# RenYurui/Global-Flow-Local-Attention

Measured on AMD Instinct MI355X. Metric: images/sec (fwd+bwd) PoseGenerator 256x176 attn_layer=2,3 -- feature-warping hot path, higher is better.
Workload: dtype f32 (FC products: 2-term f16 splits exact to 2^-24 on f16 MFMA, f32 accumulate)

## Files before the change

### global_flow_local_attention_amd/_lib.py

```python
import ctypes
import os
import subprocess

import torch

_PKG = os.path.dirname(os.path.abspath(__file__))
LIB_PATH = os.environ.get("GFLA_HIP_LIBRARY") or os.path.join(_PKG, "libgfla_hip.so")
_lib = None

_i64, _int, _ptr = ctypes.c_int64, ctypes.c_int, ctypes.c_void_p

_SIGNATURES = {
    "gfla_block_extractor_fwd": [_ptr] * 3 + [_i64] * 6 + [_int, _ptr],
    "gfla_block_extractor_bwd": [_ptr] * 5 + [_i64] * 6 + [_int, _ptr],
    "gfla_block_extractor_unfold_fwd": [_ptr] * 3 + [_i64] * 6 + [_int, _int, _ptr],
    "gfla_block_extractor_unfold_bwd": [_ptr] * 5 + [_i64] * 6 + [_int, _int, _ptr],
    "gfla_local_attn_reshape_fwd": [_ptr] * 2 + [_i64] * 3 + [_int, _ptr],
    "gfla_local_attn_reshape_bwd": [_ptr] * 2 + [_i64] * 3 + [_int, _ptr],
    "gfla_resample2d_fwd": [_ptr] * 3 + [_i64] * 6 + [_int, _int, _ptr],
    "gfla_resample2d_bwd": [_ptr] * 5 + [_i64] * 6 + [_int, _int, _int, _ptr],
    "gfla_local_attn_aggregate_fwd": [_ptr] * 5 + [_i64] * 6 + [_int, _int, _ptr],
    "gfla_local_attn_aggregate_bwd": [_ptr] * 7 + [_i64] * 6 + [_int, _int, _ptr],
    "gfla_local_attn_source_bwd": [_ptr] * 7 + [_i64] * 6 + [_int, _int, _ptr],
}
_SINGLE = {
    "gfla_max_cosine_fwd_f32": [_ptr] * 5 + [_i64] * 4 + [ctypes.c_double, _ptr],
    "gfla_max_cosine_fwd_f16": [_ptr] * 5 + [_i64] * 4 + [ctypes.c_double, _ptr],
    "gfla_max_cosine_fwd_bf16": [_ptr] * 5 + [_i64] * 4 + [ctypes.c_double, _ptr],
    "gfla_max_cosine_workspace_bytes": [_i64] * 3,
    "gfla_fc_tail_fwd_f32": [_ptr, _i64, _i64] + [_ptr] * 5 + [_i64] * 3 + [_int, ctypes.c_double, _ptr],
    "gfla_fc_tail_fwd_f64": [_ptr, _i64, _i64] + [_ptr] * 5 + [_i64] * 3 + [_int, ctypes.c_double, _ptr],
    "gfla_fc_tail_bwd_f32": [_ptr, _i64, _i64] + [_ptr] * 8 + [_i64] * 3 + [_int, ctypes.c_double, _ptr],
    "gfla_fc_tail_bwd_f64": [_ptr, _i64, _i64] + [_ptr] * 8 + [_i64] * 3 + [_int, ctypes.c_double, _ptr],
    "gfla_replicate_pad_bwd_f32": [_ptr] * 2 + [_i64] * 3 + [_int] * 4 + [_ptr],
    "gfla_replicate_pad_bwd_f64": [_ptr] * 2 + [_i64] * 3 + [_int] * 4 + [_ptr],
    "gfla_correctness_map_fwd_f32": [_ptr] * 5 + [_i64] * 3 + [ctypes.c_double] * 2 + [_ptr],
    "gfla_correctness_map_bwd_f32": [_ptr] * 9 + [_i64] * 3 + [ctypes.c_double] * 2 + [_ptr],
    "gfla_correctness_map_fwd_f16": [_ptr] * 5 + [_i64] * 3 + [ctypes.c_double] * 2 + [_ptr],
    "gfla_correctness_map_bwd_f16": [_ptr] * 9 + [_i64] * 3 + [ctypes.c_double] * 2 + [_ptr],
    "gfla_correctness_map_fwd_bf16": [_ptr] * 5 + [_i64] * 3 + [ctypes.c_double] * 2 + [_ptr],
    "gfla_correctness_map_bwd_bf16": [_ptr] * 9 + [_i64] * 3 + [ctypes.c_double] * 2 + [_ptr],
    "gfla_fc_supported": [_i64] * 3 + [_int, _int],
    "gfla_fc_workspace_bytes": [_i64] * 4 + [_int] * 3,
    "gfla_fc_forward_f32": [_ptr] * 9 + [_i64] * 4 + [_int, ctypes.c_double, _int, _ptr],
    "gfla_fc_backward_f32": [_ptr] * 12 + [_i64] * 4 + [_int, ctypes.c_double, _int, _int, _ptr],
    "gfla_fc_geometry": [_i64, _i64, _int, _int, _ptr],
    "gfla_fc_conv_fwd_f32": [_ptr, _ptr, _int, _ptr, _ptr] + [_i64] * 4 + [_int, _int, _ptr],
    "gfla_fc_conv_bwd_f32": [_ptr, _int, _ptr, _ptr, _ptr, _ptr] + [_i64] * 4 + [_int, _int, _ptr],
    "gfla_fc_tr_probe": [_ptr, _int, _ptr, _ptr, _ptr],
    "gfla_fc_wino_debug_buffer": [_ptr],
    "gfla_fc_kernel_f32": [_int, _ptr, _ptr] + [_i64] * 4 + [_int, _int, _ptr],
    "gfla_scatter_workspace_bytes": [_i64] * 3 + [_int],
    "gfla_aggregate_fwd_workspace_bytes": [_i64] * 3 + [_int],
    "gfla_aggregate_fwd_geometry": [_i64] * 6 + [_int, _ptr],
    "gfla_aggregate_bwd_supported": [_i64, _i64, _int],
    "gfla_big_plane_geometry": [_int] + [_i64] * 6 + [_int, _int, _ptr],
    "gfla_xcd_swizzle": [_i64, _i64],
    "gfla_local_attn_aggregate_fwd_ws_f32": [_ptr] * 6 + [_i64] * 6 + [_int, _int, _ptr],
    "gfla_local_attn_aggregate_fwd_ws_bf16": [_ptr] * 6 + [_i64] * 6 + [_int, _int, _ptr],
    "gfla_local_attn_aggregate_fwd_ws_f16": [_ptr] * 6 + [_i64] * 6 + [_int, _int, _ptr],
    "gfla_local_attn_aggregate_bwd_ws_f32": [_ptr] * 8 + [_i64] * 6 + [_int, _int, _ptr],
    "gfla_resample2d_bwd_ws_f32": [_ptr] * 6 + [_i64] * 6 + [_int, _int, _int, _ptr],
    "gfla_convert_multi": [_ptr, _ptr, _i64] * 4 + [_int, _ptr],
    "gfla_mask_blend_fwd_f32": [_ptr] * 6 + [_i64] * 3 + [_ptr],
    "gfla_mask_blend_fwd_bf16": [_ptr] * 6 + [_i64] * 3 + [_ptr],
    "gfla_mask_blend_bwd_f32": [_ptr] * 11 + [_i64] * 3 + [_ptr],
    "gfla_mask_blend_bwd_bf16": [_ptr] * 11 + [_i64] * 3 + [_ptr],
    "gfla_mask_blend_fwd_f16": [_ptr] * 6 + [_i64] * 3 + [_ptr],
    "gfla_mask_blend_bwd_f16": [_ptr] * 11 + [_i64] * 3 + [_ptr],
    "gfla_fc_forward_f16": [_ptr] * 9 + [_i64] * 4 + [_int, ctypes.c_double, _ptr],
    "gfla_gemm_f64_workspace_bytes": [_i64] * 3 + [_int],
    "gfla_gemm_f64": [_ptr] * 6 + [_i64] * 3 + [_int, _int, _ptr, _ptr],
    "gfla_affine_reg_workspace_bytes": [_i64] * 3 + [_int],
    "gfla_affine_reg_fwd_f32": [_ptr] * 3 + [_i64] * 3 + [_int, _ptr],
    "gfla_affine_reg_fwd_f64": [_ptr] * 3 + [_i64] * 3 + [_int, _ptr],
    "gfla_affine_reg_fwd_f16": [_ptr] * 3 + [_i64] * 3 + [_int, _ptr],
    "gfla_affine_reg_fwd_bf16": [_ptr] * 3 + [_i64] * 3 + [_int, _ptr],
    "gfla_affine_reg_bwd_f32": [_ptr] * 4 + [_i64] * 3 + [_int, _ptr],
    "gfla_affine_reg_bwd_f64": [_ptr] * 4 + [_i64] * 3 + [_int, _ptr],
    "gfla_affine_reg_bwd_f16": [_ptr] * 4 + [_i64] * 3 + [_int, _ptr],
    "gfla_affine_reg_bwd_bf16": [_ptr] * 4 + [_i64] * 3 + [_int, _ptr],
}
# ... 162 lines not shown
```

### global_flow_local_attention_amd/csrc/fc_block.hip

```cpp
#include "fc_gemm.h"

namespace gfla {

static int64_t align256(int64_t v) { return (v + 255) & ~(int64_t)255; }

enum { kAmaxSrc = 0, kAmaxTgt = 1, kAmaxW = 2, kAmaxZs = 3, kAmaxZt = 4, kAmaxSlots = 8 };

enum FcConv {
  kConvDirect,
  kConvDirect16,
  kConvWino32,
  kConvWino16,
};
enum FcWgrad {
  kWgradDirect32,
  kWgradDirect16,
  kWgradWino32,
  kWgradWino16,
};
static bool fc_wgrad_wino(FcWgrad w) { return w == kWgradWino32 || w == kWgradWino16; }

struct FcPlan {
  int split;
  bool scaled;
  FcConv fwd, dgrad;
  bool pack_wf, pack_wd;
  int pack_split;
  bool pack_uf, pack_ud;
  bool dgrads_together;
  FcWgrad wgrad;
  FcWgrad wgrad_both;
  bool wgrads_together;
  bool wgrad_x32;
// ... 527 lines not shown
  const bool unpack = L.plan.wgrad == kWgradDirect16;
  if (grad_w0 && !unpack &&
      hipMemsetAsync(grad_w0, 0, (size_t)kFcHidden * 2 * C * k * k * 4, stream) != hipSuccess)
    return GFLA_ERR_LAUNCH;
  GFLA_TRY(fc_half_backward(L, is_source != 0, ws, sc, grad_x, grad_w0, B, C, H, W, k, FcHalfCall(), stream));
  if (grad_w0 && unpack) GFLA_TRY(fc_unpack_wgrad_both(L, ws, sc, grad_w0, C, k, stream));
  return GFLA_OK;
}

int gfla_fc_kernel_f32(int which, void *workspace, void *scratch, int64_t B, int64_t C_, int64_t H_, int64_t W_,
                       int kernel_size, int mode, gfla_stream_t stream_) {
  if (!workspace || !scratch) return GFLA_ERR_NULL_POINTER;
  if (which < 0 || which > 8 || (which > 5 && !fc_is_wino(mode))) return GFLA_ERR_BAD_SHAPE;
  const int C = (int)C_, H = (int)H_, W = (int)W_, k = kernel_size;
  GFLA_TRY(fc_args_ok(B, C, H, W, k, mode));
  if (B == 0) return GFLA_OK;
  hipStream_t stream = static_cast<hipStream_t>(stream_);
  const FcLayout L = fc_layout(B, C, H, W, k, mode);
  unsigned char *ws = static_cast<unsigned char *>(workspace), *sc = static_cast<unsigned char *>(scratch);
  const bool src = which == 6 || which == 7 || (which & 1) == 0, tgt = which > 5 || (which & 1) == 1;
  float *gs = reinterpret_cast<float *>(ws + L.gs), *gt = reinterpret_cast<float *>(ws + L.gt);
  switch (which) {
    case 0: case 1: case 6: return fc_fwd_convs(L, ws, src ? gs : nullptr, tgt ? gt : nullptr, B, k, stream);
    case 2: case 3: case 7: return fc_dgrad_convs(L, ws, sc, src, tgt, B, C, k, stream);
    case 4: case 5: return fc_wgrad_half(L, src, ws, sc, B, k, stream);
    default: return fc_wgrad_wino(L.plan.wgrad_both) ? fc_wgrad_both(L, ws, sc, B, k, stream) : GFLA_ERR_UNSUPPORTED;
  }
}

int gfla_fc_tr_probe(const int16_t *image, int n_halves, const int32_t *offsets, int16_t *out, gfla_stream_t stream) {
  if (!image || !offsets || !out) return GFLA_ERR_NULL_POINTER;
  return fc_tr_probe(image, n_halves, offsets, out, static_cast<hipStream_t>(stream));
}
}
```

### global_flow_local_attention_amd/csrc/fc_wino.hip

```cpp
#include "fc_wino_shared.h"

namespace gfla {



template <int KS>
__global__ __launch_bounds__(256) void fc_wino_pack_w_kernel(const float *__restrict__ w0, WnPackJobs jobs, int C) {
  const WnPackJob jb = jobs.j[blockIdx.y];
  const int nch = (jb.n_in + kFcChunk - 1) / kFcChunk, ntn = (jb.n_out + kWnN - 1) / kWnN;
  const int64_t idx = (int64_t)blockIdx.x * 256 + threadIdx.x;
  if (!jb.U || idx >= (int64_t)ntn * kWnN * nch * kFcChunk) return;
  const int co = (int)(idx % (ntn * kWnN)), ci = (int)(idx / (ntn * kWnN));
  float w[KS][KS];
#pragma unroll
  for (int i = 0; i < KS; ++i)
#pragma unroll
    for (int j = 0; j < KS; ++j) {
      float v = 0.f;
      if (ci < jb.n_in && co < jb.n_out) {
        v = jb.dgrad ? w0[(((int64_t)ci * 2 * C + jb.c_off + co) * KS + (KS - 1 - i)) * KS + (KS - 1 - j)]
                     : w0[(((int64_t)co * 2 * C + jb.c_off + ci) * KS + i) * KS + j];
      }
      w[i][j] = v;
    }
// ... 450 lines not shown
#pragma unroll
  for (int a6 = 0; a6 < 6; ++a6) {
    if constexpr (M == 2) {
      const float a = t[a6][0], b = t[a6][1];
      zh[a6 * 6 + 0] = a, zh[a6 * 6 + 1] = a + b, zh[a6 * 6 + 2] = a - b, zh[a6 * 6 + 3] = a + 2.f * b;
      zh[a6 * 6 + 4] = a - 0.5f * b, zh[a6 * 6 + 5] = b;
    } else {
      const float a = t[a6][0], b = t[a6][1], c = t[a6][2], d = t[a6][3];
      zh[a6 * 6 + 0] = a;
      zh[a6 * 6 + 1] = a + b + c + d;
      zh[a6 * 6 + 2] = a - b + c - d;
      zh[a6 * 6 + 3] = a + 2.f * b + 4.f * c + 8.f * d;
      zh[a6 * 6 + 4] = a - 0.5f * b + 0.25f * c - 0.125f * d;
      zh[a6 * 6 + 5] = d;
    }
  }
}

struct WwUnit {
  int64_t b;
  int ty, tx0, ntx;
  int nt;
};

struct WwKArgs {
  PackedDesc X;
  const float *Z;
  float *part;
  int64_t z_bs, z_lead, total_units, SX;
  int Wp, Wo, nsplit;
  WwGeo geo;
};
template <int KS, int DBG = 0, bool MR = false>
__global__ __launch_bounds__(kWnThreads, 2) void fc_wino_wgrad_kernel(WwKArgs a0, WwKArgs a1, int nsplit0, int cpad,
                                                                     int raw_stride) {
  const bool second = (int)blockIdx.y >= nsplit0;
#define GFLA_PICK(f) (second ? a1.f : a0.f)
  PackedDesc X;
  X.base = GFLA_PICK(X.base), X.split_stride = 0, X.batch_stride = GFLA_PICK(X.batch_stride);
  X.chunk_stride = GFLA_PICK(X.chunk_stride), X.pix_stride = GFLA_PICK(X.pix_stride);
  const float *__restrict__ Z = GFLA_PICK(Z);
  float *__restrict__ part = GFLA_PICK(part);
  const int64_t z_bs = GFLA_PICK(z_bs), z_lead = GFLA_PICK(z_lead), total_units = GFLA_PICK(total_units), SX = GFLA_PICK(SX);
  const int Wp = GFLA_PICK(Wp), Wo = GFLA_PICK(Wo), nsplit = GFLA_PICK(nsplit);
  WwGeo geo;
  geo.TH = GFLA_PICK(geo.TH), geo.TW = GFLA_PICK(geo.TW), geo.nseg = GFLA_PICK(geo.nseg);
  geo.R = GFLA_PICK(geo.R), geo.ups = GFLA_PICK(geo.ups);
#undef GFLA_PICK
  constexpr int M = Ww<KS>::M, SEG = Ww<KS>::SEG, L = Ww<KS>::L, PITCH = kWwPitch;
  const int RAW = MR ? raw_stride : Ww<KS>::RAW;
  constexpr int PF1 = (6 * L * 4 + kWnThreads - 1) / kWnThreads;
  constexpr int PF = MR ? (PF1 > Ww<KS>::PFM ? PF1 : Ww<KS>::PFM) : PF1;
  extern __shared__ __attribute__((aligned(16))) unsigned char gfla_smem[];
  float *vbuf = reinterpret_cast<float *>(gfla_smem);
  unsigned char *raw = gfla_smem + 2 * kWwVFloats * 4;
  const int t = threadIdx.x, lane = t & 63, wave = t >> 6, xh = wave >> 2;
  const int cc = blockIdx.x, sp = (int)blockIdx.y - (second ? nsplit0 : 0);
  const int64_t u0 = total_units * sp / nsplit, u1 = total_units * (sp + 1) / nsplit;
  const int per_sample = geo.ups;
  const int Lr = (MR && geo.R > 1) ? M * geo.TW + 6 - M : L;
  const int raw_rows = (MR && geo.R > 1) ? M * geo.R + 6 - M : 6;
  const int npieces = raw_rows * Lr * 4;
  const unsigned inv_ntx = (65536u + (unsigned)geo.TW - 1u) / (unsigned)geo.TW;

  f32x4v acc[kWnXi];
#pragma unroll
  for (int q = 0; q < kWnXi; ++q) acc[q] = f32x4v{0.f, 0.f, 0.f, 0.f};

  auto unit_of = [&](int64_t u) {
    WwUnit un;
    un.b = u / per_sample;
    const int r = (int)(u - un.b * per_sample);
    if (MR && geo.R > 1) {
      un.ty = r * geo.R;
      un.tx0 = 0;
      un.ntx = geo.TW;
      un.nt = geo.TW * min(geo.R, geo.TH - un.ty);
    } else {
      un.ty = r / geo.nseg;
      un.tx0 = (r - un.ty * geo.nseg) * SEG;
      un.ntx = min(SEG, geo.TW - un.tx0);
      un.nt = un.ntx;
    }
    return un;
  };
  auto tile_rc = [&](int t_, int &tr, int &tcol) {
    if (MR && geo.R > 1) {
      tr = (int)(((unsigned)t_ * inv_ntx) >> 16);
      tcol = t_ - tr * geo.TW;
    } else {
// ... 220 lines not shown
constexpr int kWw16Pitch = 80;
constexpr int kWn16HeadZ = 4;
constexpr int kWw16VBytes = kWnXi * 4 * 16 * 16;

__device__ __forceinline__ void wn16_split_halves(float v, _Float16 &h, _Float16 &l) {
  asm("" : "+v"(v));
  h = (_Float16)v;
  float rem;
  asm("v_fma_mix_f32 %0, %1, 1.0, -%2 op_sel_hi:[0,0,1]" : "=v"(rem) : "v"(v), "v"(h));
  l = (_Float16)rem;
}
__device__ __forceinline__ void wn16_split_pair(float v0, float v1, uint32_t &hi, uint32_t &lo) { fc_split_pair(v0, v1, hi, lo); }
template <int A6>
__device__ __forceinline__ float ww_lift2(float a, float b) {
  if constexpr (A6 == 0) return a;
  else if constexpr (A6 == 1) return a + b;
  else if constexpr (A6 == 2) return a - b;
  else if constexpr (A6 == 3) return fmaf(2.f, b, a);
  else if constexpr (A6 == 4) return fmaf(-0.5f, b, a);
  else return b;
}

template <int A6>
__device__ __forceinline__ f32x2v ww_lift2v(f32x2v a, f32x2v b) {
  if constexpr (A6 == 0) return a;
  else if constexpr (A6 == 1) return a + b;
  else if constexpr (A6 == 2) return a - b;
  else if constexpr (A6 == 3) return __builtin_elementwise_fma(f32x2v{2.f, 2.f}, b, a);
  else if constexpr (A6 == 4) return __builtin_elementwise_fma(f32x2v{-0.5f, -0.5f}, b, a);
  else return b;
}

template <bool MR, int DBG = 0>
__global__ __launch_bounds__(kWnThreads, 2) void fc_wino16_wgrad_kernel(WwKArgs a0, WwKArgs a1, int nsplit0, int cpad,
                                                                       int raw_stride, const uint32_t *__restrict__ amax_x0,
                                                                       const uint32_t *__restrict__ amax_x1,
                                                                       const uint32_t *__restrict__ amax_z0,
                                                                       const uint32_t *__restrict__ amax_z1) {
  constexpr int KS = 5;
  const bool second = (int)blockIdx.y >= nsplit0;
#define GFLA_PICK(f) (second ? a1.f : a0.f)
  PackedDesc X;
  X.base = GFLA_PICK(X.base), X.split_stride = 0, X.batch_stride = GFLA_PICK(X.batch_stride);
  X.chunk_stride = GFLA_PICK(X.chunk_stride), X.pix_stride = GFLA_PICK(X.pix_stride);
  const float *__restrict__ Z = GFLA_PICK(Z);
  float *__restrict__ part = GFLA_PICK(part);
  const int64_t z_bs = GFLA_PICK(z_bs), z_lead = GFLA_PICK(z_lead), total_units = GFLA_PICK(total_units), SX = GFLA_PICK(SX);
  const int Wp = GFLA_PICK(Wp), nsplit = GFLA_PICK(nsplit);
  WwGeo geo;
  geo.TH = GFLA_PICK(geo.TH), geo.TW = GFLA_PICK(geo.TW), geo.nseg = GFLA_PICK(geo.nseg);
  geo.R = GFLA_PICK(geo.R), geo.ups = GFLA_PICK(geo.ups);
#undef GFLA_PICK
  const int ex = wn16_scale_exp(second ? *amax_x1 : *amax_x0, kWn16HeadX), ez = wn16_scale_exp(second ? *amax_z1 : *amax_z0, kWn16HeadZ);
  const float sx = wn16_pow2(ex), sz = wn16_pow2(ez), inv_x = wn16_pow2(254 - ex), inv_z = wn16_pow2(254 - ez);
  constexpr int M = 2, SEG = Ww<KS>::SEG, L = Ww<KS>::L, PITCH = kWw16Pitch;
  constexpr int RAW1 = (6 * L * PITCH + 15) & ~15;
  const int RAW = MR ? raw_stride : RAW1;
  constexpr int PF1 = (6 * L * 4 + kWnThreads - 1) / kWnThreads;
  constexpr int PF = MR ? (PF1 > Ww<KS>::PFM ? PF1 : Ww<KS>::PFM) : PF1;
  extern __shared__ __attribute__((aligned(16))) unsigned char gfla_smem[];
  unsigned char *vbuf = gfla_smem;
  unsigned char *raw = gfla_smem + 2 * kWw16VBytes;
  const int t = threadIdx.x, lane = t & 63, wave = t >> 6, xh = wave >> 2;
  const int cc = blockIdx.x, sp = (int)blockIdx.y - (second ? nsplit0 : 0);
  const int64_t u0 = total_units * sp / nsplit, u1 = total_units * (sp + 1) / nsplit;
  const int per_sample = geo.ups;
  const int Lr = (MR && geo.R > 1) ? M * geo.TW + 6 - M : L;
  const int raw_rows = (MR && geo.R > 1) ? M * geo.R + 6 - M : 6;
  const int npieces = raw_rows * Lr * 4;
  const unsigned inv_ntx = (65536u + (unsigned)geo.TW - 1u) / (unsigned)geo.TW;

  f32x4v acc[kWnXi];
#pragma unroll
  for (int q = 0; q < kWnXi; ++q) acc[q] = f32x4v{0.f, 0.f, 0.f, 0.f};

  auto unit_of = [&](int64_t u) {
    WwUnit un;
    un.b = u / per_sample;
    const int r = (int)(u - un.b * per_sample);
    if (MR && geo.R > 1) {
      un.ty = r * geo.R;
      un.tx0 = 0;
      un.ntx = geo.TW;
      un.nt = geo.TW * min(geo.R, geo.TH - un.ty);
    } else {
      un.ty = r / geo.nseg;
      un.tx0 = (r - un.ty * geo.nseg) * SEG;
      un.ntx = min(SEG, geo.TW - un.tx0);
      un.nt = un.ntx;
    }
    return un;
  };
  auto tile_rc = [&](int t_, int &tr, int &tcol) {
    if (MR && geo.R > 1) {
      tr = (int)(((unsigned)t_ * inv_ntx) >> 16);
      tcol = t_ - tr * geo.TW;
    } else {
// ... 257 lines not shown
  g.ups = g.R > 1 ? (g.TH + g.R - 1) / g.R : g.TH * g.nseg;
  return g;
}

int fc_wino_wgrad_splits(int64_t B, int Ho, int Wo, int cpad, int k) {
  const WwGeo g = ww_geometry(Ho, Wo, k);
  const int64_t units = B * g.ups;
  int64_t s = tuning(12) > 0 ? tuning(12) : kNumCU / (cpad / kFcChunk);
  if (s < 1) s = 1;
  return (int)(s > units ? units : s);
}

static int ww_launch(const WwJob *jobs, int njobs, int cpad, int64_t B, int k, hipStream_t stream) {
  if (k != 3 && k != 5) return GFLA_ERR_UNSUPPORTED;
  if (B <= 0 || njobs <= 0) return GFLA_OK;
  WwKArgs a[2];
  int ns[2] = {0, 0};
  bool multirow = false;
  int raw_stride = 0;
  for (int j = 0; j < 2; ++j) {
    const WwJob &J = jobs[j < njobs ? j : 0];
    if (J.X.pix_stride != 64) return GFLA_ERR_UNSUPPORTED;
    const WwGeo g = ww_geometry(J.Ho, J.Wo, k);
    const int nsplit = fc_wino_wgrad_splits(B, J.Ho, J.Wo, cpad, k);
    a[j] = WwKArgs{J.X, J.Z, J.part, J.z_bs, J.z_lead, B * g.ups, J.SX, J.Wp, J.Wo, nsplit, g};
    if (j < njobs) {
      ns[j] = nsplit;
      multirow = multirow || g.R > 1;
      const int m = k == 5 ? 2 : 4;
      const int need = g.R > 1 ? (((m * g.R + 6 - m) * (m * g.TW + 6 - m) * kWwPitch + 15) & ~15) : (k == 5 ? Ww<5>::RAW : Ww<3>::RAW);
      if (need > raw_stride) raw_stride = need;
    }
  }
  const dim3 grid((unsigned)(cpad / kFcChunk), (unsigned)(ns[0] + ns[1]));
#define GFLA_WW(K_, D_)                                                                                                \
  {                                                                                                                    \
    const unsigned lds = (unsigned)(2 * kWwVFloats * 4 + 2 * raw_stride);                                              \
    auto kern = multirow ? fc_wino_wgrad_kernel<K_, D_, true> : fc_wino_wgrad_kernel<K_, D_, false>;                   \
    (void)hipFuncSetAttribute(reinterpret_cast<const void *>(kern), hipFuncAttributeMaxDynamicSharedMemorySize, (int)lds); \
    kern<<<grid, kWnThreads, lds, stream>>>(a[0], a[1], ns[0], cpad, raw_stride);                                       \
  }
  if (k == 5) {
#ifdef GFLA_PROBES
    switch (tuning(20) >= 32 ? tuning(20) - 32 : 0) {
      case 1: GFLA_WW(5, 1) break;
      case 2: GFLA_WW(5, 2) break;
      case 4: GFLA_WW(5, 4) break;
      case 8: GFLA_WW(5, 8) break;
      case 16: GFLA_WW(5, 16) break;
      case 12: GFLA_WW(5, 12) break;
      case 29: GFLA_WW(5, 29) break;
      default: GFLA_WW(5, 0) break;
    }
#else
    GFLA_WW(5, 0)
#endif
  } else {
    GFLA_WW(3, 0)
  }
#undef GFLA_WW
  return launch_status();
}

int fc_wino_wgrad(const PackedDesc &X, const float *Z, int64_t z_bs, int64_t z_lead, float *part, int cpad, int64_t B, int Ho,
                  int Wo, int Wp, int64_t SX, int k, hipStream_t stream) {
  const WwJob job{X, Z, part, z_bs, z_lead, SX, Ho, Wo, Wp};
  return ww_launch(&job, 1, cpad, B, k, stream);
}

int fc_wino_wgrad_jobs(const WwJob *jobs, int njobs, int cpad, int64_t B, int k, hipStream_t stream) {
  if (njobs > 2) return GFLA_ERR_UNSUPPORTED;
  return ww_launch(jobs, njobs, cpad, B, k, stream);
}

int fc_wino16_wgrad_jobs(const WwJob *jobs, int njobs, int cpad, int64_t B, int k, const uint32_t *const *amax_x,
                         const uint32_t *const *amax_z, hipStream_t stream) {
  if (k != 5 || njobs > 2) return GFLA_ERR_UNSUPPORTED;
  if (B <= 0 || njobs <= 0) return GFLA_OK;
  WwKArgs a[2];
  int ns[2] = {0, 0};
  bool multirow = false;
  int raw_stride = 0;
  for (int j = 0; j < 2; ++j) {
    const int jj = j < njobs ? j : 0;
    const WwJob &J = jobs[jj];
    if (J.X.pix_stride != 64 || !amax_x[jj] || !amax_z[jj]) return GFLA_ERR_UNSUPPORTED;
    const WwGeo g = ww_geometry(J.Ho, J.Wo, k);
    const int nsplit = fc_wino_wgrad_splits(B, J.Ho, J.Wo, cpad, k);
    a[j] = WwKArgs{J.X, J.Z, J.part, J.z_bs, J.z_lead, B * g.ups, J.SX, J.Wp, J.Wo, nsplit, g};
    if (j < njobs) {
      ns[j] = nsplit;
      multirow = multirow || g.R > 1;
      const int need = g.R > 1 ? (((2 * g.R + 4) * (2 * g.TW + 4) * kWw16Pitch + 15) & ~15) : ((6 * Ww<5>::L * kWw16Pitch + 15) & ~15);
      if (need > raw_stride) raw_stride = need;
    }
  }
  const unsigned lds = (unsigned)(2 * kWw16VBytes + 2 * raw_stride);
  if (lds > kWnLdsLimit) return GFLA_ERR_UNSUPPORTED;
  const dim3 grid((unsigned)(cpad / kFcChunk), (unsigned)(ns[0] + ns[1]));
  auto kern = multirow ? fc_wino16_wgrad_kernel<true> : fc_wino16_wgrad_kernel<false>;
#ifdef GFLA_PROBES
  switch (tuning(20) >= 64 ? tuning(20) - 64 : 0) {
    case 1: kern = fc_wino16_wgrad_kernel<true, 1>; break;
    case 2: kern = fc_wino16_wgrad_kernel<true, 2>; break;
    case 3: kern = fc_wino16_wgrad_kernel<true, 3>; break;
    case 4: kern = fc_wino16_wgrad_kernel<true, 4>; break;
    case 6: kern = fc_wino16_wgrad_kernel<true, 6>; break;
    case 7: kern = fc_wino16_wgrad_kernel<true, 7>; break;
    case 8: kern = fc_wino16_wgrad_kernel<true, 8>; break;
    case 15: kern = fc_wino16_wgrad_kernel<true, 15>; break;
    default: break;
  }
#endif
  (void)hipFuncSetAttribute(reinterpret_cast<const void *>(kern), hipFuncAttributeMaxDynamicSharedMemorySize, (int)lds);
  kern<<<grid, kWnThreads, lds, stream>>>(a[0], a[1], ns[0], cpad, raw_stride, amax_x[0], amax_x[njobs > 1 ? 1 : 0], amax_z[0],
                                          amax_z[njobs > 1 ? 1 : 0]);
  return launch_status();
}


int fc_wino_wgrad_reduce(float *part, int nsplit, float *grad_w0, int C, int c_off, int cpad, int k, hipStream_t stream) {
  if (k != 3 && k != 5) return GFLA_ERR_UNSUPPORTED;
  return fc_wgrad_reduce(part, nsplit, grad_w0, C, c_off, cpad, k, stream);
}

int fc_wino_wgrad_reduce2(float *part_s, int nsplit_s, float *part_t, int nsplit_t, float *grad_w0, int C, int cpad, int k,
                          hipStream_t stream) {
  if (k != 3 && k != 5) return GFLA_ERR_UNSUPPORTED;
  return fc_wgrad_reduce2(part_s, nsplit_s, part_t, nsplit_t, grad_w0, C, cpad, k, stream);
}

}

extern "C" {
int gfla_fc_wino_debug_buffer(void *buffer) {
#ifdef GFLA_PROBES
  gfla::g_wino_stamps = static_cast<unsigned long long *>(buffer);
  return GFLA_OK;
#else
  (void)buffer;
  return GFLA_ERR_UNSUPPORTED;
#endif
}
}
```

### global_flow_local_attention_amd/csrc/fc_wino_shared.h

```cpp
#pragma once

#include "fc_gemm.h"
#include <algorithm>

namespace gfla {

constexpr int kWnXi = 36;
constexpr int kWnTiles = 32;
constexpr int kWnN = 64;
constexpr int kWnVFloats = kWnXi * kWnTiles * 8;
constexpr int kWnThreads = 512;
constexpr unsigned kWnLdsLimit = 160 * 1024;
constexpr int kWnPF = 5;

typedef float f32x2v __attribute__((ext_vector_type(2)));

template <int KS>
struct Wn {
  static constexpr int M = KS == 5 ? 2 : 4;
  static constexpr int PITCH = KS == 5 ? 80 : 72;
};

__device__ __forceinline__ void wn_bt(const float (&d)[6], float (&o)[6]) {
  o[0] = d[0] + 1.5f * d[1] - 2.f * d[2] - 1.5f * d[3] + d[4];
// ... 99 lines not shown
    if (sp < g.span) g.tpg = whole, g.span = sp;
  }
  return g;
}

template <int KS>
inline unsigned wn_raw_bytes(const WnGeo &g) { return (unsigned)((g.span * Wn<KS>::PITCH + 15) & ~15); }

template <int KS>
inline unsigned wn_lds_bytes(const WnGeo &g, bool double_raw) {
  constexpr int m = Wn<KS>::M;
  const unsigned main_loop = (unsigned)(2 * kWnVFloats * 4) + (double_raw ? 2u : 1u) * wn_raw_bytes<KS>(g);
  const unsigned exchange = (unsigned)(kWnThreads * 4 * m * m * 4);
  return main_loop > exchange ? main_loop : exchange;
}

typedef unsigned int u32x4w __attribute__((ext_vector_type(4)));
__host__ __device__ __forceinline__ int wn16_scale_exp(uint32_t amax_bits, int headroom) {
  int se = fc_scale_exp(amax_bits) - headroom;
  return se < 2 ? 2 : se;
}
__device__ __forceinline__ float wn16_pow2(int biased) { return __uint_as_float((uint32_t)biased << 23); }
constexpr int kWn16HeadX = 6, kWn16HeadW = 3;

typedef _Float16 f16x2w __attribute__((ext_vector_type(2)));
__device__ __forceinline__ uint32_t wn16_split(float v) {
  asm("" : "+v"(v));
  const _Float16 h = (_Float16)v;
  float rem;
  asm("v_fma_mix_f32 %0, %1, 1.0, -%2 op_sel_hi:[0,0,1]" : "=v"(rem) : "v"(v), "v"(h));
  return __builtin_bit_cast(uint32_t, __builtin_convertvector(f32x2v{v, rem}, f16x2w));
}

typedef float f32x4v __attribute__((ext_vector_type(4)));
typedef unsigned int u32x4v __attribute__((ext_vector_type(4)));
struct Half0 { static constexpr int value = 0; };
struct Half1 { static constexpr int value = 1; };
typedef Half1 Yes;
typedef Half0 No;

}
```

### global_flow_local_attention_amd/csrc/gfla_common.h

```cpp
#pragma once

#include <hip/hip_runtime.h>
#include <stdint.h>

#include "../../include/gfla_hip.h"

namespace gfla {

constexpr int kBlock = 256;
constexpr int kNumCU = 256;
constexpr int kNumXCD = 8;
constexpr int kWavesPerCU = 32;

struct bf16_t {
  uint16_t bits;
  bf16_t() = default;
  __host__ __device__ explicit bf16_t(float v);
  static __host__ __device__ __forceinline__ bf16_t from_bits(uint16_t b) {
    bf16_t r;
    r.bits = b;
    return r;
  }
};

// ... 44 lines not shown
  static __device__ __forceinline__ float ld(const f16_t *p) { return (float)__builtin_bit_cast(_Float16, p->bits); }
  static __host__ __device__ __forceinline__ uint16_t pack(float v) {
    return __builtin_bit_cast(uint16_t, (_Float16)v);
  }
  static __device__ __forceinline__ f16_t from(float v) { return f16_t::from_bits(pack(v)); }
};
__host__ __device__ inline f16_t::f16_t(float v) : bits(Num<f16_t>::pack(v)) {}

template <typename T, int V>
struct alignas(sizeof(T) * V) Pack {
  T v[V];
};

__device__ __forceinline__ int clampi(int v, int lo, int hi) { return max(min(v, hi), lo); }

template <typename A>
__device__ __forceinline__ A floor_t(A v);
template <>
__device__ __forceinline__ float floor_t<float>(float v) { return floorf(v); }
template <>
__device__ __forceinline__ double floor_t<double>(double v) { return floor(v); }

__device__ __forceinline__ void atomic_add(float *p, float v) {
  __hip_atomic_fetch_add(p, v, __ATOMIC_RELAXED, __HIP_MEMORY_SCOPE_AGENT);
}
__device__ __forceinline__ void atomic_add(double *p, double v) {
  __hip_atomic_fetch_add(p, v, __ATOMIC_RELAXED, __HIP_MEMORY_SCOPE_AGENT);
}
__device__ __forceinline__ void atomic_add(bf16_t *, bf16_t) { __builtin_trap(); }
__device__ __forceinline__ void atomic_add(f16_t *, f16_t) { __builtin_trap(); }

inline int64_t ceil_div(int64_t a, int64_t b) { return (a + b - 1) / b; }

inline int launch_status() {
  hipError_t e = hipGetLastError();
  return e == hipSuccess ? GFLA_OK : GFLA_ERR_LAUNCH;
}

inline int pick_channels_per_thread(int64_t threads_per_channel_group_unit, int64_t C,
                                    int64_t B, int max_cpt, int64_t want_waves = 4 * kNumCU * kWavesPerCU) {
  int cpt = max_cpt;
  while (cpt > 1) {
    int64_t groups = ceil_div(C, cpt);
    int64_t waves = threads_per_channel_group_unit * groups * B / 64;
    if (waves >= want_waves) break;
    cpt >>= 1;
  }
  return cpt < 1 ? 1 : cpt;
}

int tuning(int key);
void note_path(int id);

}
```

### global_flow_local_attention_amd/csrc/patch_mfma.hip

```cpp
#include "gfla_common.h"
#include "patch_mfma.h"
#include "rs_taps.h"

namespace gfla {

typedef float pm_f32x16 __attribute__((ext_vector_type(16)));

struct PatchEntry {
  int q;
  float v;
};

constexpr int kPmStatSlots = 32;
constexpr int kPmTile = 32;
constexpr int kPmSub = 8;
constexpr int kPmChannels = 128;
constexpr int kPmMaxNB = 6;
constexpr int kPmGPitch = 33;

struct PmLayout {
  int64_t ntiles, table_bytes, rows_bytes, total;
};
static PmLayout pm_layout(int64_t B, int64_t HW, int entries) {
  PmLayout L;
// ... 306 lines not shown
  const int pbase = tile * kPmTile + gh * 16;
#pragma unroll
  for (int q = 0; q < 4; ++q) {
    const int p = pbase + 4 * q;
    pm_f32x4 v = {0.f, 0.f, 0.f, 0.f};
    if (g_ok) {
      const float *src = g_row + (int64_t)tile * kPmTile + 4 * q;
      if (g_vec && p + 3 < HW) {
        v = *reinterpret_cast<const pm_f32x4 *>(src);
      } else {
        if (p < HW) v[0] = src[0];
        if (p + 1 < HW) v[1] = src[1];
        if (p + 2 < HW) v[2] = src[2];
        if (p + 3 < HW) v[3] = src[3];
      }
    }
    gv[q] = v;
  }
  const unsigned long long *tp = reinterpret_cast<const unsigned long long *>(tab + (int64_t)tile * kPmTile * E);
#pragma unroll
  for (int m = 0; m < kPmMaxEntriesPerThread; ++m) {
    const int e = sub + kPmSub * m;
    unsigned long long raw = 0xffffffffull;
    if (e < E) raw = tp[e];
    peq[m] = (int)(unsigned)(raw & 0xffffffffull);
    pev[m] = __uint_as_float((unsigned)(raw >> 32));
  }
}

template <int NB>
__global__ __launch_bounds__(256, 2) void patch_scatter_mfma_kernel(const float *__restrict__ G, float *__restrict__ dS,
                                                                   const PatchEntry *__restrict__ table,
                                                                   const int2 *__restrict__ tile_rows, int C, int HW,
                                                                   int Hs, int Ws, int R, int ntiles, int E,
                                                                   int accumulate, const unsigned *__restrict__ stat,
                                                                   unsigned limit) {
  constexpr int NQ = NB * 32;
  constexpr bool kSkip = NB >= 3;
  if (pm_stat_total(stat) > limit) return;
  extern __shared__ __attribute__((aligned(16))) unsigned char gfla_smem[];
  float *wt = reinterpret_cast<float *>(gfla_smem);
  float *gt = wt + kPmTile * NQ;
  unsigned short *list = reinterpret_cast<unsigned short *>(gt + kPmChannels * kPmGPitch);
  __shared__ int s_nlist;
  __shared__ unsigned s_mask[3];
  const int t = threadIdx.x, lane = t & 63, wave = t >> 6, l31 = lane & 31, kh = lane >> 5;
  const int band = blockIdx.x;
  const int64_t b = blockIdx.y;
  const int c0 = blockIdx.z * kPmChannels;
  const int by0 = band * R, by1 = min(Hs, by0 + R) - 1;
  const int nq = (by1 - by0 + 1) * Ws;

  if (wave == 0) {
    const int2 *tr = tile_rows + b * ntiles;
    int n = 0;
    for (int base = 0; base < ntiles; base += 64) {
      const int tile = base + lane;
      bool f = false;
      if (tile < ntiles) {
        const int2 rr = tr[tile];
        f = rr.x <= by1 && rr.y >= by0;
      }
      const unsigned long long m = __ballot(f);
      if (f) list[n + __popcll(m & ((1ull << lane) - 1ull))] = (unsigned short)tile;
      n += __popcll(m);
    }
    if (lane == 0) s_nlist = n;
  }
  __syncthreads();
  const int nlist = s_nlist;

  pm_f32x16 acc[NB];
#pragma unroll
  for (int j = 0; j < NB; ++j)
#pragma unroll
    for (int r = 0; r < 16; ++r) acc[j][r] = 0.f;

  const int gc = t >> 1, gh = t & 1;
  const bool g_ok = c0 + gc < C;
  const float *g_row = G + (b * C + (g_ok ? c0 + gc : 0)) * (int64_t)HW + gh * 16;
  const bool g_vec = (HW & 3) == 0 && (reinterpret_cast<uintptr_t>(G) & 15) == 0;
  const int pl = t >> 3, sub = t & (kPmSub - 1);
// ... 103 lines not shown
  (void)B, (void)C, (void)W, (void)patch;
  int R = tuning(13) > 0 ? tuning(13) : 96 / Ws;
  if (tuning(13) <= 0 && R < 2) R = (kPmMaxNB * 32) / Ws;
  if (R < 1) R = 1;
  if (R > Hs) R = Hs;
  while (R > 1 && R * Ws > kPmMaxNB * 32) --R;
  if (R * Ws > kPmMaxNB * 32) return PmGeo{0, 0, 0};
  return PmGeo{R, (int)ceil_div((int64_t)R * Ws, 32), (int)ceil_div(Hs, R)};
}

static bool pm_auto(bool aggregate, int64_t Ws) {
  if (tuning(14) == 2) return true;
  return aggregate ? true : Ws <= 24;
}

static int64_t pm_lds_bytes(int NB, int64_t ntiles) {
  return (int64_t)(kPmTile * NB * 32 + kPmChannels * kPmGPitch) * (int64_t)sizeof(float) + ((ntiles + 7) & ~(int64_t)7) * 2;
}

static bool pm_supported(int64_t B, int64_t C, int64_t H, int64_t W, int64_t Hs, int64_t Ws) {
  if (!(B > 0 && B <= 65535 && C > 0 && Hs >= 2 && Ws >= 2 && Ws <= kPmMaxNB * 32 && Hs < 32768 && Ws < 32768 &&
        H * W <= (int64_t)kPmTile * 65535 && ceil_div(C, kPmChannels) <= 65535 && tuning(14) != 1))
    return false;
  const PmGeo g = pm_geometry(B, C, (int)Hs, (int)Ws, (int)W, 0);
  return g.R > 0 && pm_lds_bytes(g.NB, ceil_div(H * W, kPmTile)) <= 64 * 1024;
}

static int pm_scatter(const float *G, float *dS, const PatchEntry *table, const int2 *tile_rows, int64_t B, int64_t C,
                      int64_t H, int64_t W, int64_t Hs, int64_t Ws, int entries, int patch, int accumulate,
                      const unsigned *stat, unsigned limit, hipStream_t stream) {
  const PmGeo g = pm_geometry(B, C, (int)Hs, (int)Ws, (int)W, patch);
  if (g.R == 0) return GFLA_ERR_UNSUPPORTED;
  const int ntiles = (int)ceil_div(H * W, kPmTile);
  const dim3 grid((unsigned)g.bands, (unsigned)B, (unsigned)ceil_div(C, kPmChannels));
  const unsigned lds = (unsigned)pm_lds_bytes(g.NB, ntiles);
  if (lds > 64 * 1024) return GFLA_ERR_UNSUPPORTED;
#define GFLA_PM(NB_)                                                                                              \
  case NB_:                                                                                                       \
    patch_scatter_mfma_kernel<NB_><<<grid, 256, lds, stream>>>(G, dS, table, tile_rows, (int)C, (int)(H * W), (int)Hs, \
                                                               (int)Ws, g.R, ntiles, entries, accumulate, stat, limit); \
    break
  switch (g.NB) {
    GFLA_PM(1);
    GFLA_PM(2);
    GFLA_PM(3);
    GFLA_PM(4);
    GFLA_PM(5);
    GFLA_PM(6);
    default: return GFLA_ERR_UNSUPPORTED;
  }
#undef GFLA_PM
  return launch_status();
}

static unsigned pm_limit(int64_t B, int64_t ntiles, int W, int patch, bool adaptive) {
  if (!adaptive || tuning(15) >= 100000) return 0xffffffffu;
  const double still = (double)kPmTile / W + 1.0 + patch;
  const double per_tile = tuning(15) > 0 ? (double)tuning(15) : 2.6 * still;
  const double total = per_tile * (double)B * (double)ntiles;
  return total >= 4.0e9 ? 0xffffffffu : (unsigned)total;
}

int agg_source_bwd_mfma(const float *flow, const float *attn, const float *gout, float *gsrc, void *workspace,
                        int64_t B, int64_t C, int64_t Hs, int64_t Ws, int64_t H, int64_t W, int k, int accumulate,
                        int adaptive, const unsigned **skip_stat, unsigned *skip_limit, hipStream_t stream) {
  if ((k != 3 && k != 5) || !pm_supported(B, C, H, W, Hs, Ws) || !workspace || !pm_auto(true, Ws)) return GFLA_ERR_UNSUPPORTED;
  const int entries = (k + 1) * (k + 1);
  const PmLayout L = pm_layout(B, H * W, entries);
  unsigned char *ws = static_cast<unsigned char *>(workspace);
  PatchEntry *table = reinterpret_cast<PatchEntry *>(ws);
  int2 *rows = reinterpret_cast<int2 *>(ws + L.table_bytes);
  unsigned *stat = reinterpret_cast<unsigned *>(ws + L.table_bytes + L.rows_bytes);
  const unsigned limit = pm_limit(B, L.ntiles, (int)W, k + 1, adaptive != 0);
// ... 61 lines not shown
```

### global_flow_local_attention_amd/csrc/tile_map.h

```cpp
#pragma once

#include "lds_plane.h"

namespace gfla {

__host__ __device__ __forceinline__ int64_t xcd_swizzle(int64_t bid, int64_t nwg) {
  const int64_t q = nwg / kNumXCD, r = nwg % kNumXCD, xcd = bid % kNumXCD;
  return (xcd < r ? xcd * (q + 1) : r * (q + 1) + (xcd - r) * q) + bid / kNumXCD;
}

__device__ __forceinline__ void box_init(int *box) {
  if (threadIdx.x == 0) {
    box[0] = box[1] = 0x7fffffff;
    box[2] = box[3] = -1;
  }
}
__device__ __forceinline__ void box_reduce(int *box, int ylo, int xlo, int yhi, int xhi) {
#pragma unroll
  for (int o = 32; o; o >>= 1) {
    ylo = min(ylo, __shfl_xor(ylo, o));
    xlo = min(xlo, __shfl_xor(xlo, o));
    yhi = max(yhi, __shfl_xor(yhi, o));
    xhi = max(xhi, __shfl_xor(xhi, o));
  }
  if ((threadIdx.x & 63) == 0) {
    atomicMin(&box[0], ylo);
    atomicMin(&box[1], xlo);
    atomicMax(&box[2], yhi);
    atomicMax(&box[3], xhi);
  }
}

struct TileWin {
  int ymin, xmin, rows, cols, size;
};
__device__ __forceinline__ TileWin tile_window(const int *box) {
  TileWin w;
  w.ymin = box[0];
  w.xmin = box[1];
  w.rows = box[2] - box[0] + 1;
  w.cols = box[3] - box[1] + 1;
  w.size = w.rows * w.cols;
// ... 185 lines not shown
```

### include/gfla_hip.h

```cpp
#ifndef GFLA_HIP_H_
#define GFLA_HIP_H_

#include <stdint.h>

#ifdef __cplusplus
extern "C" {
#endif

typedef enum gfla_status {
  GFLA_OK = 0,
  GFLA_ERR_NULL_POINTER = -1,
  GFLA_ERR_BAD_SHAPE = -2,
  GFLA_ERR_UNSUPPORTED = -3,
  GFLA_ERR_LAUNCH = -4
} gfla_status;

typedef void *gfla_stream_t;

#define GFLA_ABI_VERSION 8
int gfla_abi_version(void);
const char *gfla_status_string(int status);

int gfla_set_tuning(int key, int value);

// ... 208 lines not shown
                             const T *w1, const T *g_logits, T *g_hs, T *g_ht, T *act,              \
                             T *bias_partials, int64_t B, int64_t Hc, int64_t HW, int KK,           \
                             double slope, gfla_stream_t stream);
GFLA_DECL_FC_TAIL(f32, float)
GFLA_DECL_FC_TAIL(f64, double)
#undef GFLA_DECL_FC_TAIL

#define GFLA_FC_ACCUMULATE_SOURCE 1
#define GFLA_FC_ACCUMULATE_FLOW 2
int gfla_fc_supported(int64_t C, int64_t H, int64_t W, int kernel_size, int mode);
int64_t gfla_fc_workspace_bytes(int64_t B, int64_t C, int64_t H, int64_t W, int kernel_size, int mode,
                                int which);
int gfla_fc_forward_f32(const float *source, const float *target, const float *flow, const float *w0,
                        const float *b0, const float *w1, const float *b1, void *workspace, float *logits,
                        int64_t B, int64_t C, int64_t H, int64_t W, int kernel_size, double slope, int mode,
                        gfla_stream_t stream);
int gfla_fc_backward_f32(void *workspace, const float *flow, const float *w1, const float *grad_logits,
                         void *scratch, float *grad_source, float *grad_target, float *grad_flow, float *grad_w0,
                         float *grad_b0, float *grad_w1, float *grad_b1, int64_t B, int64_t C, int64_t H,
                         int64_t W, int kernel_size, double slope, int mode, int flags, gfla_stream_t stream);
int gfla_fc_forward_f16(const uint16_t *source, const uint16_t *target, const float *flow, const float *w0,
                        const float *b0, const float *w1, const float *b1, void *workspace, float *logits,
                        int64_t B, int64_t C, int64_t H, int64_t W, int kernel_size, double slope, gfla_stream_t stream);
int gfla_fc_geometry(int64_t H, int64_t W, int kernel_size, int is_source, int64_t *out);
int gfla_fc_conv_fwd_f32(const float *x, const float *w0, int is_source, void *workspace, float *out, int64_t B,
                         int64_t C, int64_t H, int64_t W, int kernel_size, int mode, gfla_stream_t stream);
int gfla_fc_conv_bwd_f32(const float *z, int is_source, void *workspace, void *scratch, float *grad_x,
                         float *grad_w0, int64_t B, int64_t C, int64_t H, int64_t W, int kernel_size, int mode,
                         gfla_stream_t stream);
int gfla_fc_kernel_f32(int which, void *workspace, void *scratch, int64_t B, int64_t C, int64_t H, int64_t W,
                       int kernel_size, int mode, gfla_stream_t stream);
int gfla_fc_tr_probe(const int16_t *image, int n_halves, const int32_t *offsets, int16_t *out,
                     gfla_stream_t stream);
int gfla_fc_wino_debug_buffer(void *buffer);

int gfla_replicate_pad_bwd_f32(const float *grad_padded, float *grad_in, int64_t planes, int64_t H,
                               int64_t W, int pad_left, int pad_right, int pad_top, int pad_bottom,
                               gfla_stream_t stream);
int gfla_replicate_pad_bwd_f64(const double *grad_padded, double *grad_in, int64_t planes, int64_t H,
                               int64_t W, int pad_left, int pad_right, int pad_top, int pad_bottom,
                               gfla_stream_t stream);

int64_t gfla_gemm_f64_workspace_bytes(int64_t M, int64_t N, int64_t K, int split_k);
int gfla_gemm_f64(double *c, const int64_t *c_view, const double *a, const int64_t *a_view, const double *b,
                  const int64_t *b_view, int64_t M, int64_t N, int64_t K, int beta, int split_k, void *workspace,
                  gfla_stream_t stream);

int64_t gfla_max_cosine_workspace_bytes(int64_t B, int64_t Ns, int64_t Nt);
int gfla_max_cosine_fwd_f32(const float *source, const float *target, void *workspace, float *out_max,
                            int32_t *out_idx, int64_t B, int64_t C, int64_t Ns, int64_t Nt, double eps,
                            gfla_stream_t stream);
int gfla_max_cosine_fwd_f16(const uint16_t *source, const uint16_t *target, void *workspace, float *out_max,
                            int32_t *out_idx, int64_t B, int64_t C, int64_t Ns, int64_t Nt, double eps,
                            gfla_stream_t stream);
int gfla_max_cosine_fwd_bf16(const uint16_t *source, const uint16_t *target, void *workspace, float *out_max,
                             int32_t *out_idx, int64_t B, int64_t C, int64_t Ns, int64_t Nt, double eps,
                             gfla_stream_t stream);

int gfla_correctness_map_fwd_f32(const float *warped, const float *target, const float *best,
                                 float *loss_map, float *stats, int64_t B, int64_t C, int64_t N,
                                 double eps_cos, double eps, gfla_stream_t stream);
int gfla_correctness_map_bwd_f32(const float *warped, const float *target, const float *best,
                                 const float *stats, const float *loss_map, const float *grad_map,
                                 float *grad_warped, float *grad_target, float *grad_best, int64_t B,
                                 int64_t C, int64_t N, double eps_cos, double eps, gfla_stream_t stream);
int gfla_correctness_map_fwd_f16(const float *warped, const uint16_t *target, const float *best,
// ... 60 lines not shown
```

Before: 9523.

## XCD-aware workgroup ordering for Winograd wgrad and patch scatter kernels

Replaces the 2D grid of the Winograd weight-gradient kernels with a 1D grid. Each block id maps to an XCD, and split ranges for the two jobs (source and target) are spread across XCDs, the second job in reverse XCD order, so each XCD handles a contiguous share of splits. The patch scatter MFMA kernel also moves to a 1D grid with xcd_swizzle so neighbouring bands land on the same XCD for L2 locality. This adds padding blocks that exit early when XCD shares are uneven, plus a host query function for the ordering.

```diff
diff --git a/global_flow_local_attention_amd/_lib.py b/global_flow_local_attention_amd/_lib.py
--- a/global_flow_local_attention_amd/_lib.py
+++ b/global_flow_local_attention_amd/_lib.py
@@ -48,6 +48,7 @@
     "gfla_fc_conv_fwd_f32": [_ptr, _ptr, _int, _ptr, _ptr] + [_i64] * 4 + [_int, _int, _ptr],
     "gfla_fc_conv_bwd_f32": [_ptr, _int, _ptr, _ptr, _ptr, _ptr] + [_i64] * 4 + [_int, _int, _ptr],
     "gfla_fc_tr_probe": [_ptr, _int, _ptr, _ptr, _ptr],
+    "gfla_fc_wgrad_order": [_int, _int, _int, _i64, _ptr],
     "gfla_fc_wino_debug_buffer": [_ptr],
     "gfla_fc_kernel_f32": [_int, _ptr, _ptr] + [_i64] * 4 + [_int, _int, _ptr],
     "gfla_scatter_workspace_bytes": [_i64] * 3 + [_int],
diff --git a/global_flow_local_attention_amd/csrc/fc_block.hip b/global_flow_local_attention_amd/csrc/fc_block.hip
--- a/global_flow_local_attention_amd/csrc/fc_block.hip
+++ b/global_flow_local_attention_amd/csrc/fc_block.hip
@@ -1,4 +1,5 @@
 #include "fc_gemm.h"
+#include "fc_wino_shared.h"
 
 namespace gfla {
 
@@ -592,4 +593,13 @@
   if (!image || !offsets || !out) return GFLA_ERR_NULL_POINTER;
   return fc_tr_probe(image, n_halves, offsets, out, static_cast<hipStream_t>(stream));
 }
-}
+
+int gfla_fc_wgrad_order(int nchunks, int nsplit0, int nsplit1, int64_t id, int32_t *out) {
+  if (!out) return GFLA_ERR_NULL_POINTER;
+  if (nchunks < 1 || nsplit0 < 0 || nsplit1 < 0) return GFLA_ERR_BAD_SHAPE;
+  const int64_t ids = kNumXCD * ww_order_slots(nchunks, nsplit0, nsplit1);
+  const WwSlot s = (id < 0 || id >= ids) ? WwSlot{-1, 0, 0} : ww_order(id, nchunks, nsplit0, nsplit1);
+  out[0] = s.job, out[1] = s.sp, out[2] = s.cc, out[3] = (int32_t)ids;
+  return GFLA_OK;
+}
+}
diff --git a/global_flow_local_attention_amd/csrc/fc_wino.hip b/global_flow_local_attention_amd/csrc/fc_wino.hip
--- a/global_flow_local_attention_amd/csrc/fc_wino.hip
+++ b/global_flow_local_attention_amd/csrc/fc_wino.hip
@@ -506,9 +506,11 @@
   WwGeo geo;
 };
 template <int KS, int DBG = 0, bool MR = false>
-__global__ __launch_bounds__(kWnThreads, 2) void fc_wino_wgrad_kernel(WwKArgs a0, WwKArgs a1, int nsplit0, int cpad,
-                                                                     int raw_stride) {
-  const bool second = (int)blockIdx.y >= nsplit0;
+__global__ __launch_bounds__(kWnThreads, 2) void fc_wino_wgrad_kernel(WwKArgs a0, WwKArgs a1, int nsplit0, int nsplit1,
+                                                                     int cpad, int raw_stride) {
+  const WwSlot slot = ww_order(blockIdx.x, cpad / kFcChunk, nsplit0, nsplit1);
+  if (slot.job < 0) return;
+  const bool second = slot.job == 1;
 #define GFLA_PICK(f) (second ? a1.f : a0.f)
   PackedDesc X;
   X.base = GFLA_PICK(X.base), X.split_stride = 0, X.batch_stride = GFLA_PICK(X.batch_stride);
@@ -529,7 +531,7 @@
   float *vbuf = reinterpret_cast<float *>(gfla_smem);
   unsigned char *raw = gfla_smem + 2 * kWwVFloats * 4;
   const int t = threadIdx.x, lane = t & 63, wave = t >> 6, xh = wave >> 2;
-  const int cc = blockIdx.x, sp = (int)blockIdx.y - (second ? nsplit0 : 0);
+  const int cc = slot.cc, sp = slot.sp;
   const int64_t u0 = total_units * sp / nsplit, u1 = total_units * (sp + 1) / nsplit;
   const int per_sample = geo.ups;
   const int Lr = (MR && geo.R > 1) ? M * geo.TW + 6 - M : L;
@@ -816,13 +818,15 @@
 }
 
 template <bool MR, int DBG = 0>
-__global__ __launch_bounds__(kWnThreads, 2) void fc_wino16_wgrad_kernel(WwKArgs a0, WwKArgs a1, int nsplit0, int cpad,
-                                                                       int raw_stride, const uint32_t *__restrict__ amax_x0,
+__global__ __launch_bounds__(kWnThreads, 2) void fc_wino16_wgrad_kernel(WwKArgs a0, WwKArgs a1, int nsplit0, int nsplit1,
+                                                                       int cpad, int raw_stride, const uint32_t *__restrict__ amax_x0,
                                                                        const uint32_t *__restrict__ amax_x1,
                                                                        const uint32_t *__restrict__ amax_z0,
                                                                        const uint32_t *__restrict__ amax_z1) {
   constexpr int KS = 5;
-  const bool second = (int)blockIdx.y >= nsplit0;
+  const WwSlot slot = ww_order(blockIdx.x, cpad / kFcChunk, nsplit0, nsplit1);
+  if (slot.job < 0) return;
+  const bool second = slot.job == 1;
 #define GFLA_PICK(f) (second ? a1.f : a0.f)
   PackedDesc X;
   X.base = GFLA_PICK(X.base), X.split_stride = 0, X.batch_stride = GFLA_PICK(X.batch_stride);
@@ -846,7 +850,7 @@
   unsigned char *vbuf = gfla_smem;
   unsigned char *raw = gfla_smem + 2 * kWw16VBytes;
   const int t = threadIdx.x, lane = t & 63, wave = t >> 6, xh = wave >> 2;
-  const int cc = blockIdx.x, sp = (int)blockIdx.y - (second ? nsplit0 : 0);
+  const int cc = slot.cc, sp = slot.sp;
   const int64_t u0 = total_units * sp / nsplit, u1 = total_units * (sp + 1) / nsplit;
   const int per_sample = geo.ups;
   const int Lr = (MR && geo.R > 1) ? M * geo.TW + 6 - M : L;
@@ -1170,13 +1174,13 @@
       if (need > raw_stride) raw_stride = need;
     }
   }
-  const dim3 grid((unsigned)(cpad / kFcChunk), (unsigned)(ns[0] + ns[1]));
+  const dim3 grid((unsigned)(kNumXCD * ww_order_slots(cpad / kFcChunk, ns[0], ns[1])));
 #define GFLA_WW(K_, D_)                                                                                                \
   {                                                                                                                    \
     const unsigned lds = (unsigned)(2 * kWwVFloats * 4 + 2 * raw_stride);                                              \
     auto kern = multirow ? fc_wino_wgrad_kernel<K_, D_, true> : fc_wino_wgrad_kernel<K_, D_, false>;                   \
     (void)hipFuncSetAttribute(reinterpret_cast<const void *>(kern), hipFuncAttributeMaxDynamicSharedMemorySize, (int)lds); \
-    kern<<<grid, kWnThreads, lds, stream>>>(a[0], a[1], ns[0], cpad, raw_stride);                                       \
+    kern<<<grid, kWnThreads, lds, stream>>>(a[0], a[1], ns[0], ns[1], cpad, raw_stride);                                \
   }
   if (k == 5) {
 #ifdef GFLA_PROBES
@@ -1235,7 +1239,7 @@
   }
   const unsigned lds = (unsigned)(2 * kWw16VBytes + 2 * raw_stride);
   if (lds > kWnLdsLimit) return GFLA_ERR_UNSUPPORTED;
-  const dim3 grid((unsigned)(cpad / kFcChunk), (unsigned)(ns[0] + ns[1]));
+  const dim3 grid((unsigned)(kNumXCD * ww_order_slots(cpad / kFcChunk, ns[0], ns[1])));
   auto kern = multirow ? fc_wino16_wgrad_kernel<true> : fc_wino16_wgrad_kernel<false>;
 #ifdef GFLA_PROBES
   switch (tuning(20) >= 64 ? tuning(20) - 64 : 0) {
@@ -1251,7 +1255,7 @@
   }
 #endif
   (void)hipFuncSetAttribute(reinterpret_cast<const void *>(kern), hipFuncAttributeMaxDynamicSharedMemorySize, (int)lds);
-  kern<<<grid, kWnThreads, lds, stream>>>(a[0], a[1], ns[0], cpad, raw_stride, amax_x[0], amax_x[njobs > 1 ? 1 : 0], amax_z[0],
+  kern<<<grid, kWnThreads, lds, stream>>>(a[0], a[1], ns[0], ns[1], cpad, raw_stride, amax_x[0], amax_x[njobs > 1 ? 1 : 0], amax_z[0],
                                           amax_z[njobs > 1 ? 1 : 0]);
   return launch_status();
 }
diff --git a/global_flow_local_attention_amd/csrc/fc_wino_shared.h b/global_flow_local_attention_amd/csrc/fc_wino_shared.h
--- a/global_flow_local_attention_amd/csrc/fc_wino_shared.h
+++ b/global_flow_local_attention_amd/csrc/fc_wino_shared.h
@@ -155,6 +155,32 @@
   return __builtin_bit_cast(uint32_t, __builtin_convertvector(f32x2v{v, rem}, f16x2w));
 }
 
+struct WwSlot {
+  int job, sp, cc;
+};
+__host__ __device__ __forceinline__ int ww_share_begin(int ns, int xcd) { return (int)((int64_t)ns * xcd / kNumXCD); }
+__host__ __device__ __forceinline__ WwSlot ww_order(int64_t id, int nchunks, int ns0, int ns1) {
+  const int xcd = (int)(id % kNumXCD), rx = kNumXCD - 1 - xcd;
+  const int64_t slot = id / kNumXCD;
+  int s = (int)(slot / nchunks);
+  const int cc = (int)(slot - (int64_t)s * nchunks);
+  const int b0 = ww_share_begin(ns0, xcd), n0 = ww_share_begin(ns0, xcd + 1) - b0;
+  if (s < n0) return WwSlot{0, b0 + s, cc};
+  s -= n0;
+  const int b1 = ww_share_begin(ns1, rx), n1 = ww_share_begin(ns1, rx + 1) - b1;
+  if (s < n1) return WwSlot{1, b1 + s, cc};
+  return WwSlot{-1, 0, 0};
+}
+inline int64_t ww_order_slots(int nchunks, int ns0, int ns1) {
+  int most = 0;
+  for (int x = 0; x < kNumXCD; ++x) {
+    const int rx = kNumXCD - 1 - x;
+    const int n = ww_share_begin(ns0, x + 1) - ww_share_begin(ns0, x) + ww_share_begin(ns1, rx + 1) - ww_share_begin(ns1, rx);
+    most = n > most ? n : most;
+  }
+  return (int64_t)most * nchunks;
+}
+
 typedef float f32x4v __attribute__((ext_vector_type(4)));
 typedef unsigned int u32x4v __attribute__((ext_vector_type(4)));
 struct Half0 { static constexpr int value = 0; };
diff --git a/global_flow_local_attention_amd/csrc/gfla_common.h b/global_flow_local_attention_amd/csrc/gfla_common.h
--- a/global_flow_local_attention_amd/csrc/gfla_common.h
+++ b/global_flow_local_attention_amd/csrc/gfla_common.h
@@ -100,6 +100,11 @@
 
 inline int64_t ceil_div(int64_t a, int64_t b) { return (a + b - 1) / b; }
 
+__host__ __device__ __forceinline__ int64_t xcd_swizzle(int64_t bid, int64_t nwg) {
+  const int64_t q = nwg / kNumXCD, r = nwg % kNumXCD, xcd = bid % kNumXCD;
+  return (xcd < r ? xcd * (q + 1) : r * (q + 1) + (xcd - r) * q) + bid / kNumXCD;
+}
+
 inline int launch_status() {
   hipError_t e = hipGetLastError();
   return e == hipSuccess ? GFLA_OK : GFLA_ERR_LAUNCH;
diff --git a/global_flow_local_attention_amd/csrc/patch_mfma.hip b/global_flow_local_attention_amd/csrc/patch_mfma.hip
--- a/global_flow_local_attention_amd/csrc/patch_mfma.hip
+++ b/global_flow_local_attention_amd/csrc/patch_mfma.hip
@@ -362,9 +362,9 @@
 __global__ __launch_bounds__(256, 2) void patch_scatter_mfma_kernel(const float *__restrict__ G, float *__restrict__ dS,
                                                                    const PatchEntry *__restrict__ table,
                                                                    const int2 *__restrict__ tile_rows, int C, int HW,
-                                                                   int Hs, int Ws, int R, int ntiles, int E,
-                                                                   int accumulate, const unsigned *__restrict__ stat,
-                                                                   unsigned limit) {
+                                                                   int Hs, int Ws, int R, int nbands, int ngroups,
+                                                                   int ntiles, int E, int accumulate,
+                                                                   const unsigned *__restrict__ stat, unsigned limit) {
   constexpr int NQ = NB * 32;
   constexpr bool kSkip = NB >= 3;
   if (pm_stat_total(stat) > limit) return;
@@ -375,9 +375,11 @@
   __shared__ int s_nlist;
   __shared__ unsigned s_mask[3];
   const int t = threadIdx.x, lane = t & 63, wave = t >> 6, l31 = lane & 31, kh = lane >> 5;
-  const int band = blockIdx.x;
-  const int64_t b = blockIdx.y;
-  const int c0 = blockIdx.z * kPmChannels;
+  const int64_t wg = xcd_swizzle(blockIdx.x, gridDim.x);
+  const int64_t sg = wg / nbands;
+  const int band = (int)(wg - sg * nbands);
+  const int64_t b = sg / ngroups;
+  const int c0 = (int)(sg - b * ngroups) * kPmChannels;
   const int by0 = band * R, by1 = min(Hs, by0 + R) - 1;
   const int nq = (by1 - by0 + 1) * Ws;
 
@@ -547,13 +549,15 @@
   const PmGeo g = pm_geometry(B, C, (int)Hs, (int)Ws, (int)W, patch);
   if (g.R == 0) return GFLA_ERR_UNSUPPORTED;
   const int ntiles = (int)ceil_div(H * W, kPmTile);
-  const dim3 grid((unsigned)g.bands, (unsigned)B, (unsigned)ceil_div(C, kPmChannels));
+  const int ngroups = (int)ceil_div(C, kPmChannels);
+  const int64_t nwg = (int64_t)g.bands * B * ngroups;
   const unsigned lds = (unsigned)pm_lds_bytes(g.NB, ntiles);
-  if (lds > 64 * 1024) return GFLA_ERR_UNSUPPORTED;
+  if (lds > 64 * 1024 || nwg > 0x7fffffffLL) return GFLA_ERR_UNSUPPORTED;
+  const dim3 grid((unsigned)nwg);
 #define GFLA_PM(NB_)                                                                                              \
   case NB_:                                                                                                       \
     patch_scatter_mfma_kernel<NB_><<<grid, 256, lds, stream>>>(G, dS, table, tile_rows, (int)C, (int)(H * W), (int)Hs, \
-                                                               (int)Ws, g.R, ntiles, entries, accumulate, stat, limit); \
+                                                               (int)Ws, g.R, g.bands, ngroups, ntiles, entries, accumulate, stat, limit); \
     break
   switch (g.NB) {
     GFLA_PM(1);
diff --git a/global_flow_local_attention_amd/csrc/tile_map.h b/global_flow_local_attention_amd/csrc/tile_map.h
--- a/global_flow_local_attention_amd/csrc/tile_map.h
+++ b/global_flow_local_attention_amd/csrc/tile_map.h
@@ -4,10 +4,6 @@
 
 namespace gfla {
 
-__host__ __device__ __forceinline__ int64_t xcd_swizzle(int64_t bid, int64_t nwg) {
-  const int64_t q = nwg / kNumXCD, r = nwg % kNumXCD, xcd = bid % kNumXCD;
-  return (xcd < r ? xcd * (q + 1) : r * (q + 1) + (xcd - r) * q) + bid / kNumXCD;
-}
 
 __device__ __forceinline__ void box_init(int *box) {
   if (threadIdx.x == 0) {
diff --git a/include/gfla_hip.h b/include/gfla_hip.h
--- a/include/gfla_hip.h
+++ b/include/gfla_hip.h
@@ -264,6 +264,7 @@
                        int kernel_size, int mode, gfla_stream_t stream);
 int gfla_fc_tr_probe(const int16_t *image, int n_halves, const int32_t *offsets, int16_t *out,
                      gfla_stream_t stream);
+int gfla_fc_wgrad_order(int nchunks, int nsplit0, int nsplit1, int64_t id, int32_t *out);
 int gfla_fc_wino_debug_buffer(void *buffer);
 
 int gfla_replicate_pad_bwd_f32(const float *grad_padded, float *grad_in, int64_t planes, int64_t H,
```

New measurement: 9606, median of 4. About the same (+0.9%).
